# excamera/alfalfa

Measured on AMD Instinct MI355X. Metric: 1080p macroblocks/s decode (bit-exact vs reference), higher is better.
Workload: dtype u8

## Files before the change

alfalfa_amd/csrc/kernels.hip:

```cpp
#include <hip/hip_runtime.h>
#include <algorithm>
#include <cstddef>

#include <cstdlib>

#include "device_types.h"
#include "vp8_math.hh"
#include "coeff_pack.hh"
#include "recon_inl.hh"

namespace aa {
namespace {
using namespace recon;

constexpr int kLanes = 64;

enum : int { DC_PRED, V_PRED, H_PRED, TM_PRED, B_PRED, NEARESTMV, NEARMV, ZEROMV, NEWMV, SPLITMV };

struct alignas( 16 ) ResidualLds {
  union {
    int16_t cf[25][16];
    int16_t res[24][16];
  };
  int16_t im[24][16];
// ... 762 lines not shown
    __syncthreads();

    if ( on ) {
      const int pl = l >> 3, r = l & 7;
      const uint32_t a0 = *reinterpret_cast<const uint32_t *>( &S.c[pl][0][16] ), a1 = *reinterpret_cast<const uint32_t *>( &S.c[pl][0][20] );
      const int sa = absdiff_sum4( a0 ) + absdiff_sum4( a1 );
      int sl = 0;
#pragma unroll
      for ( int i = 0; i < 8; i++ ) sl += S.c[pl][i + 1][15];
      const int dc = bigpred_dc( sa, sl, row > 0, col > 0, 3 );
      const int corner = S.c[pl][0][15], left = S.c[pl][r + 1][15];
      const int blk = 16 + pl * 4 + ( r >> 2 ) * 2;
      const uint32_t o0 = bigpred_x4( uv_mode, a0, left, corner, dc, has_res, &S.res[blk][( r & 3 ) * 4] );
      const uint32_t o1 = bigpred_x4( uv_mode, a1, left, corner, dc, has_res, &S.res[blk + 1][( r & 3 ) * 4] );
      *reinterpret_cast<uint2 *>( Cl + static_cast<size_t>( cy0 + r ) * cw + cx0 ) = make_uint2( o0, o1 );
    }
    const bool bp = on && y_mode == B_PRED;
    if ( on && !bp ) {
      const int r = l;
      uint32_t a[4];
      int sa = 0, sl = 0;
#pragma unroll
      for ( int k = 0; k < 4; k++ ) { a[k] = *reinterpret_cast<const uint32_t *>( &S.y[0][16 + 4 * k] ); sa += absdiff_sum4( a[k] ); }
#pragma unroll
      for ( int i = 0; i < 16; i++ ) sl += S.y[i + 1][15];
      const int dc = bigpred_dc( sa, sl, row > 0, col > 0, 4 );
      const int corner = S.y[0][15], left = S.y[r + 1][15];
      uint32_t o[4];
#pragma unroll
      for ( int k = 0; k < 4; k++ ) o[k] = bigpred_x4( y_mode, a[k], left, corner, dc, has_res, &S.res[( r >> 2 ) * 4 + k][( r & 3 ) * 4] );
      *reinterpret_cast<uint4 *>( Y + static_cast<size_t>( y0 + r ) * pw + x0 ) = make_uint4( o[0], o[1], o[2], o[3] );
    }
    if ( __any( bp ) ) {
#pragma unroll
      for ( int b = 0; b < 16; b++ ) {
        const int bx = b & 3, by = b >> 2;
        const int ar = by * 4, ac = bx * 4 + 15;
        if ( bp ) {
          const uint32_t word = by == 0 ? bm.x : ( by == 1 ? bm.y : ( by == 2 ? bm.z : bm.w ) );
          const int mode = ( word >> ( 8 * bx ) ) & 0xFF;
          const uint32_t e = L.tab[mode * 16 + l];
          const uint8_t * const org = &S.y[ar][ac];
          const int lift = bx == 3 ? ar * 48 : 0;
          const int e0 = org[static_cast<int>( e & 0xFF ) - ( ( e >> 24 ) & 1 ? lift : 0 )];
          const int e1 = org[static_cast<int>( ( e >> 8 ) & 0xFF ) - ( ( e >> 25 ) & 1 ? lift : 0 )];
          const int e2 = org[static_cast<int>( ( e >> 16 ) & 0xFF ) - ( ( e >> 26 ) & 1 ? lift : 0 )];
          const uint32_t above4 = *reinterpret_cast<const uint32_t *>( &S.y[ar][ac + 1] );
          const int dc = ( absdiff_sum4( above4 ) + S.y[ar + 1][ac] + S.y[ar + 2][ac] + S.y[ar + 3][ac] + S.y[ar + 4][ac] + 4 ) >> 3;
          int v = bpred_eval( e >> 27, e0, e1, e2, dc );
          if ( has_res ) v = clamp255( v + S.res[b][l] );
          S.y[ar + 1 + ( l >> 2 )][ac + 1 + ( l & 3 )] = static_cast<uint8_t>( v );
        }
        __syncthreads();
      }
      if ( bp ) *reinterpret_cast<uint4 *>( Y + static_cast<size_t>( y0 + l ) * pw + x0 ) = *reinterpret_cast<const uint4 *>( &S.y[l + 1][16] );
    }
    __syncthreads();
  }
  publish_progress( frame_on && l == 0 && !row_done, &progress[row], mbw );
}

__global__ __launch_bounds__( kLanes ) void k_recon_intra4( const aa_frame_list list, const int n_groups, const int mbh_max, aa_sync_ws * ws, const int n_xcd )
{
  __builtin_amdgcn_s_setprio( 3 );

  __shared__ Intra4Lds L;
  __shared__ int s_ticket;
  for ( int i = threadIdx.x; i < 160; i += kLanes ) {
    const uint32_t e = bpred_entry( i >> 4, i & 3, ( i >> 2 ) & 3 );
    uint32_t packed = ( e >> 24 ) << 27;
    for ( int k = 0; k < 3; k++ ) {
      const uint32_t idx = ( e >> ( 8 * k ) ) & 0xFF;
      packed |= ( idx < 4 ? ( 4 - idx ) * 48 : idx - 4 ) << ( 8 * k );
      packed |= ( idx >= 9 ? 1u : 0u ) << ( 24 + k );
    }
    L.tab[i] = packed;
  }
  const int xcc = xcc_id();
  if ( xcc >= n_xcd ) { if ( threadIdx.x == 0 ) atomicExch( &ws->error, 3 ); return; }
  for ( ;; ) {
    const int t = take_ticket( ws, xcc, &s_ticket, threadIdx.x );
    const int mine = xcc < n_groups ? ( n_groups - xcc + n_xcd - 1 ) / n_xcd : 0;
    if ( t >= mine * mbh_max ) return;
    recon_intra4_row( list, ( t % mine ) * n_xcd + xcc, t / mine, mbh_max, ws, L, xcc );
  }
}

struct alignas( 16 ) Inter4Slot {
  alignas( 16 ) int16_t res[24][16];
  union {
    struct {
      alignas( 16 ) uint8_t wy[21][24];
      uint8_t wc[2][13][16];
    };
    alignas( 16 ) uint8_t pred[384];
  };
  union {
    alignas( 16 ) uint8_t ty[16][24];
    alignas( 16 ) int16_t y2[32];
  };
  alignas( 16 ) uint8_t tc[2][8][16];
};
struct alignas( 16 ) Inter4Lds { Inter4Slot slot[4]; uint32_t taps[16]; };
static_assert( offsetof( Inter4Slot, wc ) == offsetof( Inter4Slot, wy ) + 21 * 24, "wy and wc must be contiguous" );

__device__ __forceinline__ void recon_inter4_body( const aa_dev_frame & f, const unsigned bq, const unsigned max_quads, Inter4Lds & L )
{
  const int lane = threadIdx.x, slot = lane >> 4, l = lane & 15;
  Inter4Slot & S = L.slot[slot];
  if ( lane < 16 ) {
    uint32_t a, b; pack_taps( lane >> 1, a, b ); L.taps[lane] = ( lane & 1 ) ? b : a;
  }
  const unsigned total = static_cast<unsigned>( f.mbw ) * f.mbh;
  const unsigned chunk = ( max_quads + 7u ) >> 3;
  const unsigned qi = ( bq & 7u ) * chunk + ( bq >> 3 );
  const unsigned mi = qi * 4u + slot;
  const int mbw = f.mbw, pw = mbw * 16, ph = f.mbh * 16, cw = pw >> 1, ch = ph >> 1;
  bool on = qi < max_quads && mi < total;
  const aa_mb_info * const mb = f.mbs + ( on ? mi : 0u );
  uint4 hd = make_uint4( 0, 0, 0, 0 ); uint32_t mvw = 0;
  if ( on ) { hd = *reinterpret_cast<const uint4 *>( mb ); mvw = *reinterpret_cast<const uint32_t *>( &mb->u.mv[0][0] ); }
  const int y_mode = hd.x & 0xFF, ref_frame = ( hd.x >> 16 ) & 3, segment = ( hd.x >> 24 ) & 3, flags = hd.y & 0xFF;
  const uint32_t nz_mask = hd.z, coeff_index = hd.w;
  on = on && ( flags & AA_MB_INTER ) && y_mode != SPLITMV;
  if ( !__any( on ) ) return;
  const int col = on ? static_cast<int>( mi % static_cast<unsigned>( mbw ) ) : 0, row = on ? static_cast<int>( mi / static_cast<unsigned>( mbw ) ) : 0;
  const bool has_res = on && ( flags & AA_MB_HAS_NONZERO );
  const bool has_y2 = has_res && ( flags & AA_MB_HAS_Y2 );
  const uint8_t * const * ref = f.ref[on ? ref_frame : 1];
  const uint8_t * const ref_y = ref[0], * const ref_u = ref[1], * const ref_v = ref[2];
  const int mvx = static_cast<int16_t>( mvw & 0xFFFFu ), mvy = static_cast<int>( mvw ) >> 16;
  const int cmx = chroma_mv( 4 * mvx ), cmy = chroma_mv( 4 * mvy );
  const int sxy = col * 16 + ( mvx >> 3 ) - 2, syy = row * 16 + ( mvy >> 3 ) - 2;
  const int sxc = col * 8 + ( cmx >> 3 ) - 2, syc = row * 8 + ( cmy >> 3 ) - 2;
  const int axy = sxy & ~3, axc = sxc & ~3;
  const bool inside = sxy >= 0 && syy >= 0 && axy + 24 <= pw && syy + 21 <= ph && sxc >= 0 && syc >= 0 && axc + 16 <= cw && syc + 13 <= ch;
  const bool fast = on && inside;
  uint32_t wreg[15];
  const int l6 = l / 6, lm = l - 6 * l6;
  const uint8_t * const wy0 = ref_y + static_cast<ptrdiff_t>( syy ) * pw + axy;
  const uint8_t * const wu0 = ref_u + static_cast<ptrdiff_t>( syc ) * cw + axc;
  const uint8_t * const wv0 = ref_v + static_cast<ptrdiff_t>( syc ) * cw + axc;
#pragma unroll
  for ( int k = 0; k < 15; k++ ) {
    const int i = l + 16 * k;
    wreg[k] = 0;
    if ( fast ) {
      if ( k < 7 || ( k == 7 && i < 126 ) ) {
        const int carry = lm + ( 4 * k ) % 6 >= 6 ? 1 : 0;
        const int r = l6 + 2 * k + ( 4 * k ) / 6 + carry, d = lm + ( 4 * k ) % 6 - 6 * carry;
        wreg[k] = *reinterpret_cast<const uint32_t *>( wy0 + static_cast<ptrdiff_t>( r ) * pw + d * 4 );
      } else if ( i < 230 ) {
        const int j = i - 126, pl = j >= 52 ? 1 : 0, e = j - 52 * pl;
        wreg[k] = *reinterpret_cast<const uint32_t *>( ( pl ? wv0 : wu0 ) + static_cast<ptrdiff_t>( e >> 2 ) * cw + ( e & 3 ) * 4 );
      }
    }
  }

  residual_x4( S, f, has_res, has_y2, nz_mask, coeff_index, hd.y >> 24, segment, l );

  {
    uint32_t * flat = reinterpret_cast<uint32_t *>( &S.wy[0][0] );
    if ( fast ) {
#pragma unroll
      for ( int k = 0; k < 15; k++ ) { const int i = l + 16 * k; if ( i < 230 ) flat[i] = wreg[k]; }
    }
    if ( __any( on && !inside ) ) {
      if ( on && !inside ) {
        uint8_t * by = &S.wy[0][0];
        for ( int i = l; i < 21 * 24; i += 16 ) {
          const int r = i / 24, c = i % 24;
          by[i] = ref_y[static_cast<size_t>( clampi( syy + r, 0, ph - 1 ) ) * pw + clampi( sxy + c, 0, pw - 1 )];
        }
        uint8_t * bc = &S.wc[0][0][0];
        for ( int i = l; i < 2 * 13 * 16; i += 16 ) {
          const int pl = i / 208, e = i % 208, r = e >> 4, c = e & 15;
          bc[i] = ( pl ? ref_v : ref_u )[static_cast<size_t>( clampi( syc + r, 0, ch - 1 ) ) * cw + clampi( sxc + c, 0, cw - 1 )];
        }
      }
    }
  }
  const int oy = inside ? ( sxy & 3 ) : 0, oc = inside ? ( sxc & 3 ) : 0;
  __syncthreads();

  const bool luma_general = __any( on && ( ( mvx | mvy ) & 7 ) != 0 ), chroma_general = __any( on && ( ( cmx | cmy ) & 7 ) != 0 );
  const uint8_t * const wyb = &S.wy[0][0]; const uint8_t * const wcb = &S.wc[0][0][0];
  uint8_t * const tyb = &S.ty[0][0]; uint8_t * const tcb = &S.tc[0][0][0];
  if ( on && luma_general ) {
    const int frac = mvx & 7;
    const uint32_t t0 = L.taps[2 * frac], t1 = L.taps[2 * frac + 1];
#pragma unroll
    for ( int k = 0; k < 6; k++ ) {
      const int t = l + 16 * k;
      if ( k == 5 && t >= 84 ) continue;
      const int r = t >> 2, g = t & 3;
      const uint8_t * sp = wyb + r * 24 + g * 4;
      const uint32_t o4 = sixtap_x4_lane( *reinterpret_cast<const uint32_t *>( sp ), *reinterpret_cast<const uint32_t *>( sp + 4 ), *reinterpret_cast<const uint32_t *>( sp + 8 ), oy, frac, t0, t1 );
      uint8_t * tb = tyb + ( g * 4 ) * 24 + r;
      tb[0] = static_cast<uint8_t>( o4 ); tb[24] = static_cast<uint8_t>( o4 >> 8 ); tb[48] = static_cast<uint8_t>( o4 >> 16 ); tb[72] = static_cast<uint8_t>( o4 >> 24 );
    }
  }
  if ( on && chroma_general ) {
    const int frac = cmx & 7;
    const uint32_t t0 = L.taps[2 * frac], t1 = L.taps[2 * frac + 1];
#pragma unroll
    for ( int k = 0; k < 4; k++ ) {
      const int j = l + 16 * k;
      if ( k == 3 && j >= 52 ) continue;
      const int pl = j >= 26 ? 1 : 0, e = j - 26 * pl, r = e >> 1, g = e & 1;
      const uint8_t * sp = wcb + pl * 208 + r * 16 + g * 4;
      const uint32_t o4 = sixtap_x4_lane( *reinterpret_cast<const uint32_t *>( sp ), *reinterpret_cast<const uint32_t *>( sp + 4 ), *reinterpret_cast<const uint32_t *>( sp + 8 ), oc, frac, t0, t1 );
      uint8_t * tb = tcb + pl * 128 + ( g * 4 ) * 16 + r;
      tb[0] = static_cast<uint8_t>( o4 ); tb[16] = static_cast<uint8_t>( o4 >> 8 ); tb[32] = static_cast<uint8_t>( o4 >> 16 ); tb[48] = static_cast<uint8_t>( o4 >> 24 );
    }
  }
  uint4 copy_y = make_uint4( 0, 0, 0, 0 ); uint2 copy_c = make_uint2( 0, 0 );
  if ( !luma_general && on ) {
    const uint2 * rp = reinterpret_cast<const uint2 *>( wyb + ( l + 2 ) * 24 );
    const uint2 a = rp[0], b = rp[1], c = rp[2];
    const bool q = oy + 2 >= 4; const int sft = ( oy + 2 ) & 3;
    const uint32_t e0 = q ? a.y : a.x, e1 = q ? b.x : a.y, e2 = q ? b.y : b.x, e3 = q ? c.x : b.y, e4 = q ? c.y : c.x;
    copy_y = make_uint4( __builtin_amdgcn_alignbyte( e1, e0, sft ), __builtin_amdgcn_alignbyte( e2, e1, sft ),
                         __builtin_amdgcn_alignbyte( e3, e2, sft ), __builtin_amdgcn_alignbyte( e4, e3, sft ) );
  }
  if ( !chroma_general && on ) {
    const int pl = l >> 3, r = l & 7;
    const uint2 * rp = reinterpret_cast<const uint2 *>( wcb + pl * 208 + ( r + 2 ) * 16 );
    const uint2 a = rp[0], b = rp[1];
    const bool q = oc + 2 >= 4; const int sft = ( oc + 2 ) & 3;
    const uint32_t e0 = q ? a.y : a.x, e1 = q ? b.x : a.y, e2 = q ? b.y : b.x;
    copy_c = make_uint2( __builtin_amdgcn_alignbyte( e1, e0, sft ), __builtin_amdgcn_alignbyte( e2, e1, sft ) );
  }
  __syncthreads();
  if ( !luma_general && on ) *reinterpret_cast<uint4 *>( S.pred + l * 16 ) = copy_y;
  if ( !chroma_general && on ) *reinterpret_cast<uint2 *>( S.pred + 256 + ( l >> 3 ) * 64 + ( l & 7 ) * 8 ) = copy_c;
  if ( on && luma_general ) {
    const int frac = mvy & 7;
    const uint32_t t0 = L.taps[2 * frac], t1 = L.taps[2 * frac + 1];
#pragma unroll
    for ( int k = 0; k < 4; k++ ) {
      const int t = l + 16 * k, c = t >> 2, i = t & 3;
      const uint8_t * sp = tyb + c * 24 + i * 4;
      const uint32_t o4 = sixtap_x4_lane( *reinterpret_cast<const uint32_t *>( sp ), *reinterpret_cast<const uint32_t *>( sp + 4 ), *reinterpret_cast<const uint32_t *>( sp + 8 ), 0, frac, t0, t1 );
      uint8_t * pb = S.pred + ( i * 4 ) * 16 + c;
      pb[0] = static_cast<uint8_t>( o4 ); pb[16] = static_cast<uint8_t>( o4 >> 8 ); pb[32] = static_cast<uint8_t>( o4 >> 16 ); pb[48] = static_cast<uint8_t>( o4 >> 24 );
    }
  }
  if ( on && chroma_general ) {
    const int frac = cmy & 7;
    const uint32_t t0 = L.taps[2 * frac], t1 = L.taps[2 * frac + 1];
#pragma unroll
    for ( int k = 0; k < 2; k++ ) {
      const int j = l + 16 * k, pl = j >> 4, c = ( j >> 1 ) & 7, i = j & 1;
      const uint8_t * sp = tcb + pl * 128 + c * 16 + i * 4;
      const uint32_t o4 = sixtap_x4_lane( *reinterpret_cast<const uint32_t *>( sp ), *reinterpret_cast<const uint32_t *>( sp + 4 ), *reinterpret_cast<const uint32_t *>( sp + 8 ), 0, frac, t0, t1 );
      uint8_t * pb = S.pred + 256 + pl * 64 + ( i * 4 ) * 8 + c;
      pb[0] = static_cast<uint8_t>( o4 ); pb[8] = static_cast<uint8_t>( o4 >> 8 ); pb[16] = static_cast<uint8_t>( o4 >> 16 ); pb[24] = static_cast<uint8_t>( o4 >> 24 );
    }
  }
  __syncthreads();

  if ( on ) {
    uint32_t o[4];
#pragma unroll
    for ( int k = 0; k < 4; k++ ) {
      const uint32_t p4 = *reinterpret_cast<const uint32_t *>( S.pred + l * 16 + 4 * k );
      const uint32_t out = has_res ? add_residual_x4( p4, &S.res[( l >> 2 ) * 4 + k][( l & 3 ) * 4] ) : p4;
      o[k] = out;
    }
    *reinterpret_cast<uint4 *>( f.cur[0] + static_cast<size_t>( row * 16 + l ) * pw + col * 16 ) = make_uint4( o[0], o[1], o[2], o[3] );
    const int pl = l >> 3, r = l & 7;
    uint32_t oc2[2];
#pragma unroll
    for ( int k = 0; k < 2; k++ ) {
      const uint32_t p4 = *reinterpret_cast<const uint32_t *>( S.pred + 256 + pl * 64 + r * 8 + 4 * k );
      const uint32_t out = has_res ? add_residual_x4( p4, &S.res[16 + pl * 4 + ( r >> 2 ) * 2 + k][( r & 3 ) * 4] ) : p4;
      oc2[k] = out;
    }
    *reinterpret_cast<uint2 *>( f.cur[1 + pl] + static_cast<size_t>( row * 8 + r ) * cw + col * 8 ) = make_uint2( oc2[0], oc2[1] );
  }
}

__global__ __launch_bounds__( kLanes ) void k_recon_inter4( const aa_frame_list list, const unsigned max_quads )
{
  __builtin_amdgcn_s_setprio( 3 );

  __shared__ Inter4Lds L;
  recon_inter4_body( *list.f[blockIdx.y], blockIdx.x, max_quads, L );
}

constexpr int kStripMbs = 8;
constexpr int kStripRow = 16 + 16 * kStripMbs;
constexpr int kStripRpi = 16 / kStripMbs;
static_assert( ( kStripRow / 16 ) % 2 == 1, "odd multiple of 16: consecutive rows start on different banks" );
struct alignas( 16 ) LfStrip {
  uint8_t c[12][kStripRow];
  uint8_t y[20][kStripRow];
  uint8_t halo_y[16][4];
  uint8_t halo_c[2][8][4];
  uint8_t pad[32];
};
struct alignas( 16 ) LfStripLds { LfStrip slot[4]; };

__device__ __forceinline__ uint64_t load_u64_shared( const uint8_t * p )
{
  return __hip_atomic_load( reinterpret_cast<const uint64_t *>( p ), __ATOMIC_RELAXED, __HIP_MEMORY_SCOPE_AGENT );
}

__device__ __forceinline__ void lf_edges_pk( pk2 ( &v )[20], const LfParamsPk & P, const pk2 g0, const pk2 g1, const pk2 g23 )
{
  if ( __any( g0 != 0u ) ) lf_edge_pk( P, true, g0, v[0], v[1], v[2], v[3], v[4], v[5], v[6], v[7] );
  if ( __any( g1 != 0u ) ) {
    lf_edge_pk( P, false, g1, v[4], v[5], v[6], v[7], v[8], v[9], v[10], v[11] );
    if ( __any( g23 != 0u ) ) {
      lf_edge_pk( P, false, g23, v[8], v[9], v[10], v[11], v[12], v[13], v[14], v[15] );
      lf_edge_pk( P, false, g23, v[12], v[13], v[14], v[15], v[16], v[17], v[18], v[19] );
    }
  }
}

__device__ __forceinline__ void loopfilter_strip_row( const aa_frame_list & list, const int group, const int row, const int mbh_max, const int mbw_max,
                                                       aa_sync_ws * ws, uint8_t * bnd, LfStripLds & S, const int dbg, const int home_xcc )
{
  const int lane = threadIdx.x, slot = lane >> 4, l = lane & 15;
  const aa_dev_frame & f0 = *list.f[group * 4];
  const int mbh = f0.mbh;
  if ( row >= mbh ) return;
  const aa_dev_frame * const fp = list.f[group * 4 + slot];
  const bool frame_on = fp != nullptr && fp->loop_filter_level != 0;
  if ( !__any( frame_on ) ) return;
  const aa_dev_frame & f = fp ? *fp : f0;
  LfStrip & T = S.slot[slot];
  int * const progress = ws->progress + group * mbh_max;
  const int mbw = f0.mbw, pw = mbw * 16, cw = pw >> 1;
  const int y0 = row * 16, cy0 = row * 8;
  const int sharp = f.sharpness; const bool key = f.key_frame;
  const bool last_row = row == mbh - 1;
  const bool luma = l < 8;
  const int k8 = l & 7, cp = k8 >> 2, cj = k8 & 3;
  uint8_t * const vrow = luma ? &T.y[4 + 2 * l][16] : &T.c[4 + 2 * cj][16 + 8 * kStripMbs * cp];
  uint8_t * const vhalo = luma ? &T.halo_y[2 * l][0] : &T.halo_c[cp][2 * cj][0];
  uint8_t * const hcol = luma ? &T.y[0][16 + 2 * l] : &T.c[0][16 + 8 * kStripMbs * cp + 2 * cj];
  const int mbstep = luma ? 16 : 8;
  const int brow = l / kStripMbs, bchunk = l % kStripMbs;
  uint8_t * const gy = f.cur[0] + static_cast<size_t>( y0 + brow ) * pw + 16 * bchunk;
  uint8_t * const gu = f.cur[1] + static_cast<size_t>( cy0 + brow ) * cw + 8 * bchunk;
  uint8_t * const gv = f.cur[2] + static_cast<size_t>( cy0 + brow ) * cw + 8 * bchunk;
  uint8_t * const sy = &T.y[4 + brow][16 + 16 * bchunk];
  uint8_t * const sc = &T.c[4 + brow][16 + 8 * bchunk];
  const int bl = l & 7, bq = ( bl - 4 ) & 3;
  uint8_t * const bsrc = bl < 4 ? &T.y[16 + bl][16] : &T.c[8 + 2 * ( bq & 1 )][16 + 8 * kStripMbs * ( bq >> 1 )];
  uint8_t * const btop = bl < 4 ? &T.y[bl][16] : &T.c[2 * ( bq & 1 )][16 + 8 * kStripMbs * ( bq >> 1 )];
  const int bstep = bl < 4 ? 16 : 8;
  const size_t bnd_row = ( static_cast<size_t>( group * 4 + slot ) * mbh_max + row ) * mbw_max;
  uint8_t * const bnd_own = bnd + bnd_row * 128 + 16 * bl;
  const uint8_t * const bnd_top = bnd + ( bnd_row - mbw_max ) * 128 + 16 * bl;
  const int fq = l >> 2, fr = l & 3;
  const int fix_off = fq == 0 ? 16 * fr + 12 : 64 + 32 * ( fq - 1 ) + 8 * fr + 4;
  uint8_t * const fix_src0 = fq == 0 ? &T.halo_y[12 + fr][0] : &T.halo_c[( fq - 1 ) & 1][4 + fr][0];
  uint8_t * const fix_srck = fq == 0 ? &T.y[16 + fr][16 - 4] : &T.c[8 + fr][16 + 8 * kStripMbs * ( ( fq - 1 ) & 1 ) - 4];
  const int fix_step = fq == 0 ? 16 : 8;
  uint8_t * const fy = f.cur[0] + static_cast<size_t>( y0 + l ) * pw - 4;
  uint8_t * const fc = f.cur[1 + ( l >> 3 )] + static_cast<size_t>( cy0 + ( l & 7 ) ) * cw - 4;
  const aa_mb_info * const mbrow = f.mbs + static_cast<size_t>( row ) * mbw;

  const int n_strips = ( mbw + kStripMbs - 1 ) / kStripMbs;
  uint4 py[kStripMbs]; uint2 pc[kStripMbs];
#pragma unroll
  for ( int i = 0; i < kStripMbs; i++ ) { py[i] = make_uint4( 0, 0, 0, 0 ); pc[i] = make_uint2( 0, 0 ); }
  auto prefetch = [&]( const int s ) {
    const bool in = frame_on && !( dbg & 2 ) && s * kStripMbs + bchunk < mbw;
    if ( in ) {
#pragma unroll
      for ( int i = 0; i < kStripMbs; i++ ) py[i] = *reinterpret_cast<const uint4 *>( gy + static_cast<size_t>( kStripRpi * i ) * pw + 16 * kStripMbs * s );
#pragma unroll
      for ( int i = 0; i < kStripMbs / 2; i++ ) pc[i] = *reinterpret_cast<const uint2 *>( gu + static_cast<size_t>( kStripRpi * i ) * cw + 8 * kStripMbs * s );
#pragma unroll
      for ( int i = 0; i < kStripMbs / 2; i++ ) pc[kStripMbs / 2 + i] = *reinterpret_cast<const uint2 *>( gv + static_cast<size_t>( kStripRpi * i ) * cw + 8 * kStripMbs * s );
    }
  };
  prefetch( 0 );
  int info = frame_on ? *reinterpret_cast<const uint16_t *>( &mbrow[0].flags ) : 0;
  int seen = row > 0 ? 0 : mbw;
  LfParamsPk P = lf_params_pk( lf_params( 1, sharp, key ) );
  int p_level = -1;
  for ( int s = 0; s < n_strips; s++ ) {
    const int nmb = min( kStripMbs, mbw - s * kStripMbs );
    if ( s > 0 ) {
      *reinterpret_cast<uint32_t *>( &T.halo_y[l][0] ) = *reinterpret_cast<const uint32_t *>( &T.y[4 + l][16 + 16 * kStripMbs - 4] );
      *reinterpret_cast<uint32_t *>( &T.halo_c[l >> 3][l & 7][0] ) = *reinterpret_cast<const uint32_t *>( &T.c[4 + ( l & 7 )][16 + 8 * kStripMbs * ( l >> 3 ) + 8 * kStripMbs - 4] );
      __syncthreads();
    }
#pragma unroll
    for ( int i = 0; i < kStripMbs; i++ ) *reinterpret_cast<uint4 *>( sy + kStripRpi * kStripRow * i ) = py[i];
#pragma unroll
    for ( int i = 0; i < kStripMbs / 2; i++ ) { *reinterpret_cast<uint2 *>( sc + kStripRpi * kStripRow * i ) = pc[i]; *reinterpret_cast<uint2 *>( sc + kStripRpi * kStripRow * i + 8 * kStripMbs ) = pc[kStripMbs / 2 + i]; }
    __syncthreads();

    for ( int k = 0; k < nmb; k++ ) {
      const int col = s * kStripMbs + k;
      const int level = info >> 8;
      const bool active = level != 0;
      const bool inner = !( info & AA_MB_LF_SKIP_INNER );
      const bool more = col + 1 < mbw;
      const int info_next = ( frame_on && more ) ? *reinterpret_cast<const uint16_t *>( &mbrow[col + 1].flags ) : 0;
      const int need = col + 1;
      if ( row > 0 && seen < need ) seen = poll_progress( &progress[row - 1] );
      const bool any_active = __any( active );
      if ( !__all( level == p_level ) ) { P = lf_params_pk( lf_params( active ? level : 1, sharp, key ) ); p_level = level; }
      const pk2 g_on = active ? ~0u : 0u, g_in = ( active && inner ) ? ~0u : 0u, g_in23 = ( active && inner && luma ) ? ~0u : 0u;

      if ( any_active && !( dbg & 4 ) ) {
        uint8_t * const ra = vrow + mbstep * k;
        uint8_t * const ha = k == 0 ? vhalo : ra - 4;
        uint8_t * const hb = k == 0 ? vhalo + 4 : ra + kStripRow - 4;
        uint32_t a[5], b[5];
        a[0] = *reinterpret_cast<const uint32_t *>( ha ); b[0] = *reinterpret_cast<const uint32_t *>( hb );
        { const uint2 u = *reinterpret_cast<const uint2 *>( ra ); a[1] = u.x; a[2] = u.y; }
        { const uint2 u = *reinterpret_cast<const uint2 *>( ra + 8 ); a[3] = u.x; a[4] = u.y; }
        { const uint2 u = *reinterpret_cast<const uint2 *>( ra + kStripRow ); b[1] = u.x; b[2] = u.y; }
        { const uint2 u = *reinterpret_cast<const uint2 *>( ra + kStripRow + 8 ); b[3] = u.x; b[4] = u.y; }
        pk2 v[20];
#pragma unroll
        for ( int d = 0; d < 5; d++ ) {
          v[4 * d] = pk_from_bytes<0>( a[d], b[d] ); v[4 * d + 1] = pk_from_bytes<1>( a[d], b[d] );
          v[4 * d + 2] = pk_from_bytes<2>( a[d], b[d] ); v[4 * d + 3] = pk_from_bytes<3>( a[d], b[d] );
        }
        lf_edges_pk( v, P, col > 0 ? g_on : 0u, g_in, g_in23 );
#pragma unroll
        for ( int d = 0; d < 5; d++ ) pk_to_dwords( v[4 * d], v[4 * d + 1], v[4 * d + 2], v[4 * d + 3], a[d], b[d] );
        if ( active ) {
          *reinterpret_cast<uint32_t *>( ha ) = a[0]; *reinterpret_cast<uint32_t *>( hb ) = b[0];
          *reinterpret_cast<uint2 *>( ra ) = make_uint2( a[1], a[2] ); *reinterpret_cast<uint2 *>( ra + kStripRow ) = make_uint2( b[1], b[2] );
          if ( luma ) { *reinterpret_cast<uint2 *>( ra + 8 ) = make_uint2( a[3], a[4] ); *reinterpret_cast<uint2 *>( ra + kStripRow + 8 ) = make_uint2( b[3], b[4] ); }
        }
      }
      __syncthreads();
      if ( frame_on && !last_row && col > 0 && l < 12 && !( dbg & 1 ) ) {
        const uint8_t * src = k == 0 ? fix_src0 : fix_srck + fix_step * k;
        *reinterpret_cast<uint32_t *>( bnd + ( bnd_row + col - 1 ) * 128 + fix_off ) = *reinterpret_cast<const uint32_t *>( src );
      }

      if ( row > 0 ) {
        if ( !( dbg & 16 ) ) wait_for_row_above( true, need, seen, 2, ws, progress, group, row, mbh, home_xcc, lf_min_polls( dbg ), lf_max_wait_ticks( dbg ) );

        if ( frame_on && l < 8 && !( dbg & 8 ) ) {
          const uint8_t * src = bnd_top + static_cast<size_t>( col ) * 128;
          const uint64_t lo = load_u64_shared( src ), hi = load_u64_shared( src + 8 );
          uint8_t * dst = btop + bstep * k;
          if ( bl < 4 ) { *reinterpret_cast<uint64_t *>( dst ) = lo; *reinterpret_cast<uint64_t *>( dst + 8 ) = hi; }
          else { *reinterpret_cast<uint64_t *>( dst ) = lo; *reinterpret_cast<uint64_t *>( dst + kStripRow ) = hi; }
        }
      }
      publish_progress( lane == 0 && col > 0 && !lf_fault_injected( dbg, row ), &progress[row], col );
      if ( k == 0 && s + 1 < n_strips ) prefetch( s + 1 );
      __syncthreads();

      if ( any_active && !( dbg & 4 ) ) {
        uint8_t * const hc = hcol + mbstep * k;
        pk2 v[20];
#pragma unroll
        for ( int r = 0; r < 20; r++ ) v[r] = pk_from_u16( *reinterpret_cast<const uint16_t *>( hc + kStripRow * r ) );
        lf_edges_pk( v, P, row > 0 ? g_on : 0u, g_in, g_in23 );
        if ( active ) {
#pragma unroll
          for ( int r = 1; r < 12; r++ ) *reinterpret_cast<uint16_t *>( hc + kStripRow * r ) = static_cast<uint16_t>( pk_to_u16( v[r] ) );
          if ( luma ) {
#pragma unroll
            for ( int r = 12; r < 20; r++ ) *reinterpret_cast<uint16_t *>( hc + kStripRow * r ) = static_cast<uint16_t>( pk_to_u16( v[r] ) );
          }
        }
      }
      __syncthreads();

      if ( frame_on && !( dbg & 1 ) ) {
        if ( !last_row ) {
          if ( l < 8 ) {
            const uint8_t * src = bsrc + bstep * k;
            uint4 q;
            if ( bl < 4 ) q = *reinterpret_cast<const uint4 *>( src );
            else { const uint2 u0 = *reinterpret_cast<const uint2 *>( src ), u1 = *reinterpret_cast<const uint2 *>( src + kStripRow ); q = make_uint4( u0.x, u0.y, u1.x, u1.y ); }
            *reinterpret_cast<uint4 *>( bnd_own + static_cast<size_t>( col ) * 128 ) = q;
          }
        }
        if ( k == 0 && s > 0 ) {
          if ( l < 12 || last_row ) *reinterpret_cast<uint32_t *>( fy + 16 * kStripMbs * s ) = *reinterpret_cast<const uint32_t *>( &T.halo_y[l][0] );
          if ( ( l & 7 ) < 4 || last_row ) *reinterpret_cast<uint32_t *>( fc + 8 * kStripMbs * s ) = *reinterpret_cast<const uint32_t *>( &T.halo_c[l >> 3][l & 7][0] );
        }
        if ( k == nmb - 1 && bchunk < nmb ) {
#pragma unroll
          for ( int i = 0; i < 20 / kStripRpi; i++ ) {
            if ( ( ( i + 1 ) * kStripRpi > 4 || row > 0 ) && ( i * kStripRpi < 16 || last_row ) )
              *reinterpret_cast<uint4 *>( gy + ( static_cast<ptrdiff_t>( kStripRpi * i ) - 4 ) * pw + 16 * kStripMbs * s ) = *reinterpret_cast<const uint4 *>( sy + kStripRpi * kStripRow * i - 4 * kStripRow );
          }
#pragma unroll
          for ( int i = 0; i < 12 / kStripRpi; i++ ) {
            if ( ( ( i + 1 ) * kStripRpi > 4 || row > 0 ) && ( i * kStripRpi < 8 || last_row ) ) {
              *reinterpret_cast<uint2 *>( gu + ( static_cast<ptrdiff_t>( kStripRpi * i ) - 4 ) * cw + 8 * kStripMbs * s ) = *reinterpret_cast<const uint2 *>( sc + kStripRpi * kStripRow * i - 4 * kStripRow );
              *reinterpret_cast<uint2 *>( gv + ( static_cast<ptrdiff_t>( kStripRpi * i ) - 4 ) * cw + 8 * kStripMbs * s ) = *reinterpret_cast<const uint2 *>( sc + kStripRpi * kStripRow * i - 4 * kStripRow + 8 * kStripMbs );
            }
          }
        }
      }
      info = info_next;
      __syncthreads();
    }
  }
  publish_progress( lane == 0 && !lf_fault_injected( dbg, row ), &progress[row], mbw );
}

__device__ __forceinline__ void loopfilter_rows4_body( const aa_frame_list & list, const int n_groups, const int mbh_max, const int mbw_max, aa_sync_ws * ws, uint8_t * bnd,
                                                        const int n_xcd, LfStripLds & S, int & s_ticket, const int dbg )
{
  const int xcc = xcc_id();
  if ( xcc >= n_xcd ) { if ( threadIdx.x == 0 ) atomicExch( &ws->error, 3 ); return; }
  for ( ;; ) {
    const int t = take_ticket( ws, xcc, &s_ticket, threadIdx.x );
    const int mine = xcc < n_groups ? ( n_groups - xcc + n_xcd - 1 ) / n_xcd : 0;
    if ( t >= mine * mbh_max ) return;
    loopfilter_strip_row( list, ( t % mine ) * n_xcd + xcc, t / mine, mbh_max, mbw_max, ws, bnd, S, dbg, xcc );
  }
}

__global__ __launch_bounds__( kLanes ) __attribute__( ( amdgpu_waves_per_eu( 2 ) ) ) void k_loopfilter_rows4( const aa_frame_list list, const int n_groups, const int mbh_max, const int mbw_max, aa_sync_ws * ws, uint8_t * bnd,
                                                                 const int n_xcd, const int dbg )
{
  __builtin_amdgcn_s_setprio( 3 );

  __shared__ LfStripLds S;
  __shared__ int s_ticket;
  loopfilter_rows4_body( list, n_groups, mbh_max, mbw_max, ws, bnd, n_xcd, S, s_ticket, dbg );
}

__global__ void k_probe_xcds( int * out )
{
  if ( threadIdx.x == 0 ) atomicAdd( &out[xcc_id() & 15], 1 );
}

__global__ void k_probe_concurrency( uint32_t * counter, uint32_t * seen, uint32_t n, unsigned long long timeout, int slot )
{
  if ( threadIdx.x || blockIdx.x ) return;
  __hip_atomic_fetch_add( counter, 1u, __ATOMIC_RELAXED, __HIP_MEMORY_SCOPE_AGENT );
  const unsigned long long t0 = wall_clock64();
  uint32_t m;
  while ( ( m = __hip_atomic_load( counter, __ATOMIC_RELAXED, __HIP_MEMORY_SCOPE_AGENT ) ) < n && wall_clock64() - t0 < timeout ) __builtin_amdgcn_s_sleep( 32 );
  seen[slot] = m;
}

__global__ void k_check_tickets( aa_sync_ws * ws, const int n_groups, const int mbh_max, const int n_xcd )
{
  if ( threadIdx.x != 0 || blockIdx.x != 0 ) return;
  for ( int x = 0; x < n_xcd; x++ ) {
    const int mine = x < n_groups ? ( n_groups - x + n_xcd - 1 ) / n_xcd : 0;
    const int t = __hip_atomic_load( &ws->ticket[x], __ATOMIC_RELAXED, __HIP_MEMORY_SCOPE_AGENT );
    if ( t < mine * mbh_max && atomicCAS( &ws->error, 0, 5 ) == 0 ) { ws->where[0] = x; ws->where[1] = t; ws->where[2] = mine * mbh_max; }
  }
}

__global__ void k_bind_rasters( const aa_raster_binding * b, int n )
{
  const int i = blockIdx.x * blockDim.x + threadIdx.x;
  if ( i >= n ) return;
  aa_dev_frame * f = b[i].job;
  for ( int p = 0; p < 3; p++ ) f->cur[p] = b[i].cur[p];
  for ( int r = 1; r < 4; r++ ) for ( int p = 0; p < 3; p++ ) f->ref[r][p] = b[i].ref[r - 1][p];
}

__global__ __launch_bounds__( 256 ) void k_gather_rasters( const aa_gather_job * jobs, uint8_t * staging, size_t stride )
{
  const aa_gather_job J = jobs[blockIdx.y];
  const uint4 * src = reinterpret_cast<const uint4 *>( J.src );
  uint4 * dst = reinterpret_cast<uint4 *>( staging + stride * blockIdx.y );
  const size_t n16 = J.bytes >> 4;
  for ( size_t i = size_t( blockIdx.x ) * 256 + threadIdx.x; i < n16; i += size_t( gridDim.x ) * 256 ) dst[i] = src[i];
  if ( blockIdx.x == 0 && threadIdx.x < ( J.bytes & 15 ) ) staging[stride * blockIdx.y + ( n16 << 4 ) + threadIdx.x] = J.src[( n16 << 4 ) + threadIdx.x];
}

constexpr int kRgbCy = 76309, kRgbCrv = 104574, kRgbCgu = 25642, kRgbCgv = 53281, kRgbCbu = 132213;

template <int ESZ, int N>
__device__ inline void rgb_store( uint8_t * p, const uint32_t ( &e )[N], const int n, const bool fast )
{
  static_assert( ( N * ESZ ) % 16 == 0, "whole 16-byte pieces" );
  if ( fast ) {
    uint32_t w[N * ESZ / 4];
#pragma unroll
    for ( int i = 0; i < N * ESZ / 4; i++ ) {
      if ( ESZ == 1 ) w[i] = e[4 * i] | e[4 * i + 1] << 8 | e[4 * i + 2] << 16 | e[4 * i + 3] << 24;
      else if ( ESZ == 2 ) w[i] = ( e[2 * i] & 0xFFFFu ) | e[2 * i + 1] << 16;
      else w[i] = e[i];
    }
    uint4 * q = reinterpret_cast<uint4 *>( p );
#pragma unroll
    for ( int i = 0; i < N * ESZ / 16; i++ ) q[i] = make_uint4( w[4 * i], w[4 * i + 1], w[4 * i + 2], w[4 * i + 3] );
    return;
  }
#pragma unroll
  for ( int i = 0; i < N; i++ )
    if ( i < n )
#pragma unroll
      for ( int b = 0; b < ESZ; b++ ) p[i * ESZ + b] = static_cast<uint8_t>( e[i] >> ( 8 * b ) );
}

template <int F>
__global__ __launch_bounds__( 256 ) void k_render_rgb( const aa_rgb_job * jobs, const uint32_t * table )
{
  constexpr bool kFloat = F >= AA_RGB_F16_CHW;
  constexpr int kEsz = F == AA_RGB_F32_CHW ? 4 : F >= AA_RGB_F16_CHW ? 2 : 1;
  __shared__ uint32_t T[kFloat ? 768 : 1];
  if ( kFloat ) {
    for ( int i = threadIdx.x; i < 768; i += 256 ) T[i] = table[i];
    __syncthreads();
  }
  const aa_rgb_job & J = jobs[blockIdx.y];
  const uint32_t groups = J.groups, w = J.width, h = J.height;
  const uint32_t t = blockIdx.x * 256u + threadIdx.x;
  if ( t >= groups * ( ( h + 1 ) >> 1 ) ) return;
  const int k = static_cast<int>( t / groups ), x0 = static_cast<int>( t - uint32_t( k ) * groups ) * 16;
  const int cw = static_cast<int>( ( w + 1 ) >> 1 ), ch = static_cast<int>( ( h + 1 ) >> 1 );
  const int j0 = x0 >> 1, je = min( j0 + 8, cw - 1 );
  const int crow[3] = { max( k - 1, 0 ), k, min( k + 1, ch - 1 ) };
  int c[2][3][9];
#pragma unroll
  for ( int p = 0; p < 2; p++ )
#pragma unroll
    for ( int r = 0; r < 3; r++ ) {
      const uint8_t * row = J.plane[1 + p] + size_t( crow[r] ) * J.stride_c;
      const uint2 q = *reinterpret_cast<const uint2 *>( row + j0 );
      c[p][r][8] = row[je];
#pragma unroll
      for ( int i = 0; i < 8; i++ ) {
        const int b = static_cast<int>( ( ( i < 4 ? q.x : q.y ) >> ( 8 * ( i & 3 ) ) ) & 255u );
        c[p][r][i] = j0 + i > je ? c[p][r][8] : b;
      }
    }
  const int n = min( 16, static_cast<int>( w ) - x0 );
  for ( int r = 0; r < 2; r++ ) {
    const int y = 2 * k + r;
    if ( y >= static_cast<int>( h ) ) continue;
    const uint4 yq = *reinterpret_cast<const uint4 *>( J.plane[0] + size_t( y ) * J.stride_y + x0 );
    const uint32_t yw[4] = { yq.x, yq.y, yq.z, yq.w };
    int v[2][9];
#pragma unroll
    for ( int p = 0; p < 2; p++ )
#pragma unroll
      for ( int i = 0; i < 9; i++ ) v[p][i] = 3 * c[p][1][i] + c[p][r ? 2 : 0][i];
    uint32_t R[16], G[16], B[16];
#pragma unroll
    for ( int i = 0; i < 16; i++ ) {
      const int Y = static_cast<int>( ( yw[i >> 2] >> ( 8 * ( i & 3 ) ) ) & 255u );
      const int j = i >> 1;
      const int u8 = ( i & 1 ) ? v[0][j] + v[0][j + 1] : 2 * v[0][j];
      const int v8 = ( i & 1 ) ? v[1][j] + v[1][j + 1] : 2 * v[1][j];
      const int yt = 8 * kRgbCy * ( Y - 16 ), ut = u8 - 1024, vt = v8 - 1024;
      R[i] = static_cast<uint32_t>( min( max( ( yt + kRgbCrv * vt + ( 1 << 18 ) ) >> 19, 0 ), 255 ) );
      G[i] = static_cast<uint32_t>( min( max( ( yt - kRgbCgu * ut - kRgbCgv * vt + ( 1 << 18 ) ) >> 19, 0 ), 255 ) );
      B[i] = static_cast<uint32_t>( min( max( ( yt + kRgbCbu * ut + ( 1 << 18 ) ) >> 19, 0 ), 255 ) );
    }
    uint8_t * const row = J.dst + y * J.row_stride;
    if ( F == AA_RGB_U8_HWC3 || F == AA_RGB_U8_HWC4 ) {
      constexpr int C = F == AA_RGB_U8_HWC3 ? 3 : 4;
      uint32_t e[16 * C];
#pragma unroll
      for ( int i = 0; i < 16; i++ ) {
        e[C * i] = R[i]; e[C * i + 1] = G[i]; e[C * i + 2] = B[i];
        if ( C == 4 ) e[C * i + 3] = 255u;
      }
      uint8_t * const p = row + x0 * C;
      rgb_store<1, 16 * C>( p, e, n * C, n == 16 && !( reinterpret_cast<uintptr_t>( p ) & 15 ) );
    } else {
#pragma unroll
      for ( int ci = 0; ci < 3; ci++ ) {
        const uint32_t * const src = ci == 0 ? R : ci == 1 ? G : B;
        uint32_t e[16];
#pragma unroll
        for ( int i = 0; i < 16; i++ ) e[i] = kFloat ? T[ci * 256 + src[i]] : src[i];
        uint8_t * const p = row + ci * J.plane_stride + x0 * kEsz;
        rgb_store<kEsz, 16>( p, e, n, n == 16 && !( reinterpret_cast<uintptr_t>( p ) & 15 ) );
      }
    }
  }
}

}

__global__ __launch_bounds__( 256 ) void k_lf_relevel( const aa_mb_info * src, aa_mb_info * dst, unsigned nmb, uint32_t levels )
{
  const unsigned i = blockIdx.x * blockDim.x + threadIdx.x;
  if ( i >= nmb ) return;
  const uint4 * s = reinterpret_cast<const uint4 *>( src + i );
  uint4 * d = reinterpret_cast<uint4 *>( dst + i );
  uint4 head = s[0];
  const uint32_t seg = ( head.x >> 24 ) & 3u;
  head.y = ( head.y & 0xFFFF00FFu ) | ( ( ( levels >> ( 8 * seg ) ) & 255u ) << 8 );
  d[0] = head;
  for ( int k = 1; k < 5; k++ ) d[k] = s[k];
}
static_assert( sizeof( aa_mb_info ) == 80, "k_lf_relevel copies five 16-byte pieces" );

int launch_lf_relevel( const aa_mb_info * src, aa_mb_info * dst, unsigned nmb, uint32_t levels, void * stream )
{
  hipLaunchKernelGGL( k_lf_relevel, dim3( ( nmb + 255 ) / 256 ), dim3( 256 ), 0, static_cast<hipStream_t>( stream ), src, dst, nmb, levels );
  return static_cast<int>( hipGetLastError() );
}

int launch_gather_rasters( const aa_gather_job * jobs, int n, uint8_t * staging, size_t stride, size_t max_bytes, void * stream )
{
  const unsigned per = static_cast<unsigned>( std::min<size_t>( 64, std::max<size_t>( 1, max_bytes / ( 256 * 16 * 4 ) ) ) );
  for ( int base = 0; base < n; base += 32768 ) {
    const int cnt = std::min( 32768, n - base );
    hipLaunchKernelGGL( k_gather_rasters, dim3( per, cnt ), dim3( 256 ), 0, static_cast<hipStream_t>( stream ), jobs + base, staging + stride * base, stride );
    if ( hipError_t e = hipGetLastError() ) return static_cast<int>( e );
  }
  return 0;
}

int launch_render_rgb( const aa_rgb_job * jobs, int n, int format, const uint32_t * table, uint32_t max_threads, void * stream )
{
  const unsigned blocks = ( max_threads + 255u ) / 256u;
  const hipStream_t st = static_cast<hipStream_t>( stream );
  for ( int base = 0; base < n; base += 32768 ) {
    const dim3 grid( blocks, std::min( 32768, n - base ) );
    switch ( format ) {
      case AA_RGB_U8_HWC3: hipLaunchKernelGGL( k_render_rgb<AA_RGB_U8_HWC3>, grid, dim3( 256 ), 0, st, jobs + base, table ); break;
      case AA_RGB_U8_HWC4: hipLaunchKernelGGL( k_render_rgb<AA_RGB_U8_HWC4>, grid, dim3( 256 ), 0, st, jobs + base, table ); break;
      case AA_RGB_U8_CHW: hipLaunchKernelGGL( k_render_rgb<AA_RGB_U8_CHW>, grid, dim3( 256 ), 0, st, jobs + base, table ); break;
      case AA_RGB_F16_CHW: hipLaunchKernelGGL( k_render_rgb<AA_RGB_F16_CHW>, grid, dim3( 256 ), 0, st, jobs + base, table ); break;
      case AA_RGB_BF16_CHW: hipLaunchKernelGGL( k_render_rgb<AA_RGB_BF16_CHW>, grid, dim3( 256 ), 0, st, jobs + base, table ); break;
      case AA_RGB_F32_CHW: hipLaunchKernelGGL( k_render_rgb<AA_RGB_F32_CHW>, grid, dim3( 256 ), 0, st, jobs + base, table ); break;
      default: return static_cast<int>( hipErrorInvalidValue );
    }
    if ( hipError_t e = hipGetLastError() ) return static_cast<int>( e );
  }
  return 0;
}

int launch_bind_rasters( const aa_raster_binding * b, int n, void * stream )
{
  hipLaunchKernelGGL( k_bind_rasters, dim3( ( n + 63 ) / 64 ), dim3( 64 ), 0, static_cast<hipStream_t>( stream ), b, n );
  return static_cast<int>( hipGetLastError() );
}

int launch_recon_inter( const aa_frame_list & list, int n, unsigned max_mbs, bool split_only, void * stream )
{
  const unsigned blocks = ( ( max_mbs + 7u ) >> 3 ) * 8u;
  hipLaunchKernelGGL( k_recon_inter, dim3( blocks, n ), dim3( kLanes ), 0, static_cast<hipStream_t>( stream ), list, max_mbs, split_only ? 1 : 0 );
  return static_cast<int>( hipGetLastError() );
}
int launch_recon_inter4( const aa_frame_list & list, int n, unsigned max_mbs, void * stream )
{
  const unsigned quads = ( max_mbs + 3u ) >> 2;
  const unsigned blocks = ( ( quads + 7u ) >> 3 ) * 8u;
  hipLaunchKernelGGL( k_recon_inter4, dim3( blocks, n ), dim3( kLanes ), 0, static_cast<hipStream_t>( stream ), list, quads );
  return static_cast<int>( hipGetLastError() );
}
int launch_recon_intra_diagonal( const aa_frame_list & list, int n, int diagonal, int row_lo, int rows, void * stream )
{
  hipLaunchKernelGGL( k_recon_intra, dim3( rows, n ), dim3( kLanes ), 0, static_cast<hipStream_t>( stream ), list, diagonal, row_lo );
  return static_cast<int>( hipGetLastError() );
}
int launch_loopfilter_diagonal( const aa_frame_list & list, int n, int diagonal, int row_lo, int rows, void * stream )
{
  hipLaunchKernelGGL( k_loopfilter, dim3( rows, n ), dim3( kLanes ), 0, static_cast<hipStream_t>( stream ), list, diagonal, row_lo );
  return static_cast<int>( hipGetLastError() );
}
static int lf_debug_bits()
{
  static const int bits = [] { const char * e = std::getenv( "ALFALFA_AMD_LF_DEBUG" ); return e ? std::atoi( e ) : 0; }();
  return bits;
}
static unsigned test_lds_pad()
{
  static const unsigned pad = [] { const char * e = std::getenv( "ALFALFA_AMD_TEST_LDS_PAD" ); return e ? static_cast<unsigned>( std::atoi( e ) ) : 0u; }();
  return pad;
}
int launch_loopfilter_rows4( const aa_frame_list & list, int n_groups, int mbh_max, int mbw_max, aa_sync_ws * ws, uint8_t * boundary, int n_xcd, void * stream )
{
  hipLaunchKernelGGL( k_loopfilter_rows4, dim3( n_xcd * ( ( n_groups + n_xcd - 1 ) / n_xcd ) * mbh_max ), dim3( kLanes ), test_lds_pad(), static_cast<hipStream_t>( stream ), list, n_groups, mbh_max, mbw_max, ws, boundary, n_xcd, lf_debug_bits() );
  hipLaunchKernelGGL( k_check_tickets, dim3( 1 ), dim3( 64 ), 0, static_cast<hipStream_t>( stream ), ws, n_groups, mbh_max, n_xcd );
  return static_cast<int>( hipGetLastError() );
}
int launch_recon_intra4( const aa_frame_list & list, int n_groups, int mbh_max, aa_sync_ws * ws, int n_xcd, void * stream )
{
  hipLaunchKernelGGL( k_recon_intra4, dim3( n_xcd * ( ( n_groups + n_xcd - 1 ) / n_xcd ) * mbh_max ), dim3( kLanes ), test_lds_pad(), static_cast<hipStream_t>( stream ), list, n_groups, mbh_max, ws, n_xcd );
  hipLaunchKernelGGL( k_check_tickets, dim3( 1 ), dim3( 64 ), 0, static_cast<hipStream_t>( stream ), ws, n_groups, mbh_max, n_xcd );
  return static_cast<int>( hipGetLastError() );
}
int launch_probe_concurrency( uint32_t * counter, uint32_t * seen, uint32_t n, unsigned long long timeout_ticks, int slot, void * stream )
{
  hipLaunchKernelGGL( k_probe_concurrency, dim3( 1 ), dim3( 64 ), 0, static_cast<hipStream_t>( stream ), counter, seen, n, timeout_ticks, slot );
  return static_cast<int>( hipGetLastError() );
}
int launch_probe_xcds( int * out16, int blocks, void * stream )
{
  hipLaunchKernelGGL( k_probe_xcds, dim3( blocks ), dim3( kLanes ), 0, static_cast<hipStream_t>( stream ), out16 );
  return static_cast<int>( hipGetLastError() );
}

}
```

Baseline: 124.7 million.

## Prefetch above-row boundary early and tag frame pointers as global address space

Frame and mode-info pointers in the loop-filter strip kernel are cast to address space 1, so the compiler can emit global instead of flat memory instructions. The top-boundary load is split across all 16 lanes at 8 bytes each instead of 8 lanes at 16 bytes. When the row-above progress is already known to be far enough ahead, that load is issued before the filtering work so its latency overlaps it. Otherwise the kernel falls back to the wait-then-load path. This adds a wave-wide vote and some branching per macroblock, and the early load depends on the progress check being correct.

Result: no change. 125.8 million, median of 6 (+0.9%).

```diff
diff --git a/alfalfa_amd/csrc/kernels.hip b/alfalfa_amd/csrc/kernels.hip
--- a/alfalfa_amd/csrc/kernels.hip
+++ b/alfalfa_amd/csrc/kernels.hip
@@ -1088,6 +1088,13 @@
 };
 struct alignas( 16 ) LfStripLds { LfStrip slot[4]; };
 
+#if defined( __HIP_DEVICE_COMPILE__ )
+#define LF_HBM __attribute__( ( address_space( 1 ) ) )
+#else
+#define LF_HBM
+#endif
+template <typename T> __device__ __forceinline__ LF_HBM T * in_hbm( T * p ) { return reinterpret_cast<LF_HBM T *>( reinterpret_cast<uintptr_t>( p ) ); }
+
 __device__ __forceinline__ uint64_t load_u64_shared( const uint8_t * p )
 {
   return __hip_atomic_load( reinterpret_cast<const uint64_t *>( p ), __ATOMIC_RELAXED, __HIP_MEMORY_SCOPE_AGENT );
@@ -1129,26 +1136,27 @@
   uint8_t * const hcol = luma ? &T.y[0][16 + 2 * l] : &T.c[0][16 + 8 * kStripMbs * cp + 2 * cj];
   const int mbstep = luma ? 16 : 8;
   const int brow = l / kStripMbs, bchunk = l % kStripMbs;
-  uint8_t * const gy = f.cur[0] + static_cast<size_t>( y0 + brow ) * pw + 16 * bchunk;
-  uint8_t * const gu = f.cur[1] + static_cast<size_t>( cy0 + brow ) * cw + 8 * bchunk;
-  uint8_t * const gv = f.cur[2] + static_cast<size_t>( cy0 + brow ) * cw + 8 * bchunk;
+  LF_HBM uint8_t * const gy = in_hbm( f.cur[0] ) + static_cast<size_t>( y0 + brow ) * pw + 16 * bchunk;
+  LF_HBM uint8_t * const gu = in_hbm( f.cur[1] ) + static_cast<size_t>( cy0 + brow ) * cw + 8 * bchunk;
+  LF_HBM uint8_t * const gv = in_hbm( f.cur[2] ) + static_cast<size_t>( cy0 + brow ) * cw + 8 * bchunk;
   uint8_t * const sy = &T.y[4 + brow][16 + 16 * bchunk];
   uint8_t * const sc = &T.c[4 + brow][16 + 8 * bchunk];
   const int bl = l & 7, bq = ( bl - 4 ) & 3;
   uint8_t * const bsrc = bl < 4 ? &T.y[16 + bl][16] : &T.c[8 + 2 * ( bq & 1 )][16 + 8 * kStripMbs * ( bq >> 1 )];
-  uint8_t * const btop = bl < 4 ? &T.y[bl][16] : &T.c[2 * ( bq & 1 )][16 + 8 * kStripMbs * ( bq >> 1 )];
   const int bstep = bl < 4 ? 16 : 8;
+  uint8_t * const btop = l < 8 ? &T.y[l >> 1][16 + 8 * ( l & 1 )] : &T.c[l & 3][16 + 8 * kStripMbs * ( ( l >> 2 ) & 1 )];
+  const int tstep = l < 8 ? 16 : 8;
   const size_t bnd_row = ( static_cast<size_t>( group * 4 + slot ) * mbh_max + row ) * mbw_max;
-  uint8_t * const bnd_own = bnd + bnd_row * 128 + 16 * bl;
-  const uint8_t * const bnd_top = bnd + ( bnd_row - mbw_max ) * 128 + 16 * bl;
+  uint8_t * const bnd_line = bnd + bnd_row * 128;
+  const int own_off = 16 * bl, top_off = 8 * l - 128 * mbw_max;
   const int fq = l >> 2, fr = l & 3;
   const int fix_off = fq == 0 ? 16 * fr + 12 : 64 + 32 * ( fq - 1 ) + 8 * fr + 4;
   uint8_t * const fix_src0 = fq == 0 ? &T.halo_y[12 + fr][0] : &T.halo_c[( fq - 1 ) & 1][4 + fr][0];
   uint8_t * const fix_srck = fq == 0 ? &T.y[16 + fr][16 - 4] : &T.c[8 + fr][16 + 8 * kStripMbs * ( ( fq - 1 ) & 1 ) - 4];
   const int fix_step = fq == 0 ? 16 : 8;
-  uint8_t * const fy = f.cur[0] + static_cast<size_t>( y0 + l ) * pw - 4;
-  uint8_t * const fc = f.cur[1 + ( l >> 3 )] + static_cast<size_t>( cy0 + ( l & 7 ) ) * cw - 4;
-  const aa_mb_info * const mbrow = f.mbs + static_cast<size_t>( row ) * mbw;
+  LF_HBM uint8_t * const fy = in_hbm( f.cur[0] ) + static_cast<size_t>( y0 + l ) * pw - 4;
+  LF_HBM uint8_t * const fc = in_hbm( f.cur[1 + ( l >> 3 )] ) + static_cast<size_t>( cy0 + ( l & 7 ) ) * cw - 4;
+  const LF_HBM aa_mb_info * const mbrow = in_hbm( f.mbs ) + static_cast<size_t>( row ) * mbw;
 
   const int n_strips = ( mbw + kStripMbs - 1 ) / kStripMbs;
   uint4 py[kStripMbs]; uint2 pc[kStripMbs];
@@ -1158,15 +1166,15 @@
     const bool in = frame_on && !( dbg & 2 ) && s * kStripMbs + bchunk < mbw;
     if ( in ) {
 #pragma unroll
-      for ( int i = 0; i < kStripMbs; i++ ) py[i] = *reinterpret_cast<const uint4 *>( gy + static_cast<size_t>( kStripRpi * i ) * pw + 16 * kStripMbs * s );
-#pragma unroll
-      for ( int i = 0; i < kStripMbs / 2; i++ ) pc[i] = *reinterpret_cast<const uint2 *>( gu + static_cast<size_t>( kStripRpi * i ) * cw + 8 * kStripMbs * s );
-#pragma unroll
-      for ( int i = 0; i < kStripMbs / 2; i++ ) pc[kStripMbs / 2 + i] = *reinterpret_cast<const uint2 *>( gv + static_cast<size_t>( kStripRpi * i ) * cw + 8 * kStripMbs * s );
+      for ( int i = 0; i < kStripMbs; i++ ) py[i] = *reinterpret_cast<const LF_HBM uint4 *>( gy + static_cast<size_t>( kStripRpi * i ) * pw + 16 * kStripMbs * s );
+#pragma unroll
+      for ( int i = 0; i < kStripMbs / 2; i++ ) pc[i] = *reinterpret_cast<const LF_HBM uint2 *>( gu + static_cast<size_t>( kStripRpi * i ) * cw + 8 * kStripMbs * s );
+#pragma unroll
+      for ( int i = 0; i < kStripMbs / 2; i++ ) pc[kStripMbs / 2 + i] = *reinterpret_cast<const LF_HBM uint2 *>( gv + static_cast<size_t>( kStripRpi * i ) * cw + 8 * kStripMbs * s );
     }
   };
   prefetch( 0 );
-  int info = frame_on ? *reinterpret_cast<const uint16_t *>( &mbrow[0].flags ) : 0;
+  int info = frame_on ? *reinterpret_cast<const LF_HBM uint16_t *>( &mbrow[0].flags ) : 0;
   int seen = row > 0 ? 0 : mbw;
   LfParamsPk P = lf_params_pk( lf_params( 1, sharp, key ) );
   int p_level = -1;
@@ -1189,8 +1197,13 @@
       const bool active = level != 0;
       const bool inner = !( info & AA_MB_LF_SKIP_INNER );
       const bool more = col + 1 < mbw;
-      const int info_next = ( frame_on && more ) ? *reinterpret_cast<const uint16_t *>( &mbrow[col + 1].flags ) : 0;
+      const int info_next = ( frame_on && more ) ? *reinterpret_cast<const LF_HBM uint16_t *>( &mbrow[col + 1].flags ) : 0;
       const int need = col + 1;
+      const bool top_on = frame_on && !( dbg & 8 );
+      const uint8_t * const top_src = bnd_line + static_cast<ptrdiff_t>( col * 128 + top_off );
+      uint64_t top = 0;
+      const bool ahead = row > 0 && __all( seen >= need );
+      if ( ahead && top_on ) top = load_u64_shared( top_src );
       if ( row > 0 && seen < need ) seen = poll_progress( &progress[row - 1] );
       const bool any_active = __any( active );
       if ( !__all( level == p_level ) ) { P = lf_params_pk( lf_params( active ? level : 1, sharp, key ) ); p_level = level; }
@@ -1222,21 +1235,15 @@
         }
       }
       __syncthreads();
+      if ( ahead && top_on ) *reinterpret_cast<uint64_t *>( btop + tstep * k ) = top;
       if ( frame_on && !last_row && col > 0 && l < 12 && !( dbg & 1 ) ) {
         const uint8_t * src = k == 0 ? fix_src0 : fix_srck + fix_step * k;
-        *reinterpret_cast<uint32_t *>( bnd + ( bnd_row + col - 1 ) * 128 + fix_off ) = *reinterpret_cast<const uint32_t *>( src );
-      }
-
-      if ( row > 0 ) {
+        *reinterpret_cast<uint32_t *>( bnd_line + ( ( col - 1 ) * 128 + fix_off ) ) = *reinterpret_cast<const uint32_t *>( src );
+      }
+
+      if ( row > 0 && !ahead ) {
         if ( !( dbg & 16 ) ) wait_for_row_above( true, need, seen, 2, ws, progress, group, row, mbh, home_xcc, lf_min_polls( dbg ), lf_max_wait_ticks( dbg ) );
-
-        if ( frame_on && l < 8 && !( dbg & 8 ) ) {
-          const uint8_t * src = bnd_top + static_cast<size_t>( col ) * 128;
-          const uint64_t lo = load_u64_shared( src ), hi = load_u64_shared( src + 8 );
-          uint8_t * dst = btop + bstep * k;
-          if ( bl < 4 ) { *reinterpret_cast<uint64_t *>( dst ) = lo; *reinterpret_cast<uint64_t *>( dst + 8 ) = hi; }
-          else { *reinterpret_cast<uint64_t *>( dst ) = lo; *reinterpret_cast<uint64_t *>( dst + kStripRow ) = hi; }
-        }
+        if ( top_on ) *reinterpret_cast<uint64_t *>( btop + tstep * k ) = load_u64_shared( top_src );
       }
       publish_progress( lane == 0 && col > 0 && !lf_fault_injected( dbg, row ), &progress[row], col );
       if ( k == 0 && s + 1 < n_strips ) prefetch( s + 1 );
@@ -1266,24 +1273,24 @@
             uint4 q;
             if ( bl < 4 ) q = *reinterpret_cast<const uint4 *>( src );
             else { const uint2 u0 = *reinterpret_cast<const uint2 *>( src ), u1 = *reinterpret_cast<const uint2 *>( src + kStripRow ); q = make_uint4( u0.x, u0.y, u1.x, u1.y ); }
-            *reinterpret_cast<uint4 *>( bnd_own + static_cast<size_t>( col ) * 128 ) = q;
+            *reinterpret_cast<uint4 *>( bnd_line + ( col * 128 + own_off ) ) = q;
           }
         }
         if ( k == 0 && s > 0 ) {
-          if ( l < 12 || last_row ) *reinterpret_cast<uint32_t *>( fy + 16 * kStripMbs * s ) = *reinterpret_cast<const uint32_t *>( &T.halo_y[l][0] );
-          if ( ( l & 7 ) < 4 || last_row ) *reinterpret_cast<uint32_t *>( fc + 8 * kStripMbs * s ) = *reinterpret_cast<const uint32_t *>( &T.halo_c[l >> 3][l & 7][0] );
+          if ( l < 12 || last_row ) *reinterpret_cast<LF_HBM uint32_t *>( fy + 16 * kStripMbs * s ) = *reinterpret_cast<const uint32_t *>( &T.halo_y[l][0] );
+          if ( ( l & 7 ) < 4 || last_row ) *reinterpret_cast<LF_HBM uint32_t *>( fc + 8 * kStripMbs * s ) = *reinterpret_cast<const uint32_t *>( &T.halo_c[l >> 3][l & 7][0] );
         }
         if ( k == nmb - 1 && bchunk < nmb ) {
 #pragma unroll
           for ( int i = 0; i < 20 / kStripRpi; i++ ) {
             if ( ( ( i + 1 ) * kStripRpi > 4 || row > 0 ) && ( i * kStripRpi < 16 || last_row ) )
-              *reinterpret_cast<uint4 *>( gy + ( static_cast<ptrdiff_t>( kStripRpi * i ) - 4 ) * pw + 16 * kStripMbs * s ) = *reinterpret_cast<const uint4 *>( sy + kStripRpi * kStripRow * i - 4 * kStripRow );
+              *reinterpret_cast<LF_HBM uint4 *>( gy + ( static_cast<ptrdiff_t>( kStripRpi * i ) - 4 ) * pw + 16 * kStripMbs * s ) = *reinterpret_cast<const uint4 *>( sy + kStripRpi * kStripRow * i - 4 * kStripRow );
           }
 #pragma unroll
           for ( int i = 0; i < 12 / kStripRpi; i++ ) {
             if ( ( ( i + 1 ) * kStripRpi > 4 || row > 0 ) && ( i * kStripRpi < 8 || last_row ) ) {
-              *reinterpret_cast<uint2 *>( gu + ( static_cast<ptrdiff_t>( kStripRpi * i ) - 4 ) * cw + 8 * kStripMbs * s ) = *reinterpret_cast<const uint2 *>( sc + kStripRpi * kStripRow * i - 4 * kStripRow );
-              *reinterpret_cast<uint2 *>( gv + ( static_cast<ptrdiff_t>( kStripRpi * i ) - 4 ) * cw + 8 * kStripMbs * s ) = *reinterpret_cast<const uint2 *>( sc + kStripRpi * kStripRow * i - 4 * kStripRow + 8 * kStripMbs );
+              *reinterpret_cast<LF_HBM uint2 *>( gu + ( static_cast<ptrdiff_t>( kStripRpi * i ) - 4 ) * cw + 8 * kStripMbs * s ) = *reinterpret_cast<const uint2 *>( sc + kStripRpi * kStripRow * i - 4 * kStripRow );
+              *reinterpret_cast<LF_HBM uint2 *>( gv + ( static_cast<ptrdiff_t>( kStripRpi * i ) - 4 ) * cw + 8 * kStripMbs * s ) = *reinterpret_cast<const uint2 *>( sc + kStripRpi * kStripRow * i - 4 * kStripRow + 8 * kStripMbs );
             }
           }
         }
```
